# TAMUCrypto/virgo-plus

Measured on AMD Instinct MI355X. Metric: prover sec + field-ops/sec, SHA-256 circuit, 1/2/4/8 MI355X (bit-exact), higher is better.
Workload: dtype u64 (F_p^2, p=2^61-1); 1 GPU; SHA-256 1024-block circuit (SHA256_64.pws x1024, 102347776 gates, 15 layers, 2^23 input wires), GKR sumcheck + Virgo FFT/LDT commit on GPU (BASELINE configs[2]); pass_mode=sync, field_ops_per_proof=8299342697

## Files before the change

### virgo-plus_amd/__init__.py

```python
import ctypes
import os
import shutil
import subprocess

PKG_DIR = os.path.dirname(os.path.abspath(__file__))
ROOT = os.path.dirname(PKG_DIR)
CSRC = os.path.join(PKG_DIR, "csrc")
HOST = os.path.join(PKG_DIR, "host")
LIB_GPU = os.environ.get("VP_LIBGPU") or os.path.join(CSRC, "libvpgpu.so")
LIB_GPU_CHECKED = os.path.join(ROOT, "tools", "_build", "checked", "libvpgpu.so")
LIB_GPU_TESTDRV = os.path.join(ROOT, "tools", "_build", "testdrv", "libvpgpu.so")
LIB_HOST = os.path.join(HOST, "libvphost.so")
CLI = os.path.join(HOST, "virgo_plus_run")

GPU_SRC = [os.path.join(CSRC, f) for f in ("vpgpu.hip", "vpgpu_batched.inc", "vpgpu_pc.inc", "vpgpu_pc_shard.inc", "vpgpu_fftgkr.inc", "vpgpu_upload.inc", "vp_kernels_fftgkr.h", "vp_kernels.h", "vp_kernels_round.h", "vp_kernels_persist.h", "vp_kernels_batch.h",
                                              "vp_kernels_plan.h", "vp_kernels_pc.h", "vp_kernels_ntt8.h", "vp_kernels_ntt_long.h", "vp_keccak_asm.h", "vp_check.h", "vp_field.h", "vp_fri_layout.h", "vp_pc_live.h", "vp_pc_corners.h")] + [
    os.path.join(ROOT, "include", "vpgpu.h")]
HOST_SRC = [os.path.join(HOST, f) for f in ("circuit.cpp", "prover.cpp", "verifier.cpp", "vphost.cpp")]
HOST_HDR = [os.path.join(HOST, f) for f in ("circuit.hpp", "prover.hpp", "verifier.hpp", "vphost.h", "field.hpp",
                                              "polynomial.hpp")]


def _stale(target, sources):
    if not os.path.exists(target):
# ... 547 lines not shown
                                                1 if skip_predicates else 0) == 0

    def verify_full_record(self, record):
        buf = ctypes.create_string_buffer(bytes(record), max(len(record), 1))
        return lib_host().vph_verify_full_record(self.h, ctypes.cast(buf, ctypes.c_void_p), len(record)) == 0

    def verify_fs(self, proof):
        buf = ctypes.create_string_buffer(bytes(proof), len(proof))
        return lib_host().vph_verify_fs(self.h, ctypes.cast(buf, ctypes.c_void_p), len(proof)) == 0

    def close(self):
        if self.h:
            lib_host().vph_circuit_free(self.h)
            self.h = None


_PUBLIC_OPTIONS = ("use_graph", "plan_autotune", "real_values", "real_pairs", "pc_tensor_pub", "persistent_rounds", "persistent_timeout_ms", "poll", "prefetch_round1",
                   "interactive_fast_init", "split_cost_percent", "debug")
_TUNING_ENV = {"gkr_path": "VP_GKR_PATH", "serial": "VP_GKR_SERIAL", "fuse_init": "VP_FUSE_INIT", "fuse_min_log": "VP_FUSE_MIN_LOG", "fuse_dot": "VP_FUSE_DOT",
               "drop_y": "VP_DROP_Y", "drop_y_round1": "VP_DROP_Y1", "seg_tiny": "VP_SEG_TINY", "sf_big_log": "VP_SF_BIG_LOG", "sf3b_grid": "VP_SF3B_GRID",
               "dot_blocks": "VP_DOT_BLOCKS", "plan_align": "VP_PLAN_ALIGN", "round_fused_max": "VP_ROUND_FUSED_MAX",
               "kernel_copies": "VP_KERNEL_COPIES", "fold_branches": "VP_FOLD_BRANCHES", "fuse_combine": "VP_FUSE_COMBINE",
               "graph_explicit": "VP_GRAPH_EXPLICIT", "ntt_r8": "VP_NTT_R8", "fuse_p2": "VP_FUSE_P2", "leaf_asm": "VP_LEAF_ASM",
               "fft_gkr_batched": "VP_FFT_GKR_BATCHED", "split_vu": "VP_SPLIT_VU", "pc_live": "VP_PC_LIVE"}
VP_OPTIONS_ABI = 0x76700005


class Options(ctypes.Structure):
    _fields_ = [("struct_size", ctypes.c_uint32), ("abi", ctypes.c_uint32)] + [(n, ctypes.c_int32) for n in _PUBLIC_OPTIONS] + [("reserved", ctypes.c_int32 * 4)]

    def __init__(self, **kw):
        super().__init__()
        lib_gpu().vp_options_default(ctypes.byref(self))
        self.tuning = {}
        for k, v in kw.items():
            if k in _PUBLIC_OPTIONS:
                setattr(self, k, v)
            elif k in _TUNING_ENV:
                self.tuning[k] = v
            else:
                raise TypeError("unknown option " + k)

    def tuning_env(self):
        env = {}
        for k, v in getattr(self, "tuning", {}).items():
            if k == "gkr_path":
                v = {PATH_PLAN: "plan", PATH_LANES: "lanes", PATH_SIMPLE: "simple"}[v]
# ... 431 lines not shown
```

### virgo-plus_amd/csrc/vp_kernels_ntt8.h

```cpp
#pragma once

namespace vp {

constexpr u64 LZ_P2 = 2 * P61;
constexpr u64 LZ_P4 = 4 * P61;
__device__ __forceinline__ u64 lz_fold(u64 x) { return (x & P61) + (x >> 61); }
__device__ __forceinline__ F lz_fold(const F &x) { return f_make(lz_fold(x.re), lz_fold(x.im)); }
__device__ __forceinline__ F lz_add(const F &a, const F &b) { return f_make(a.re + b.re, a.im + b.im); }
template <u64 K> __device__ __forceinline__ F lz_sub(const F &a, const F &b) { return f_make(a.re + (K - b.re), a.im + (K - b.im)); }
template <bool INV, u64 K> __device__ __forceinline__ F lz_mul_w4(const F &x) { return INV ? f_make(K - x.im, x.re) : f_make(x.im, K - x.re); }
__device__ __forceinline__ u64 lz_rot30(u64 v) { return (v >> 31) + ((v & 0x7fffffffull) << 30); }
template <bool INV> __device__ __forceinline__ F lz_mul_w8(const F &x) {
    const u64 s = x.re + x.im;
    return INV ? f_make(lz_rot30(x.re + (LZ_P2 - x.im)), lz_rot30(s)) : f_make(lz_rot30(s), lz_rot30(x.im + (LZ_P2 - x.re)));
}
__device__ __forceinline__ F lz_canon(const F &x) {
    u64 a = lz_fold(x.re), b = lz_fold(x.im);
    return f_make(a >= P61 ? a - P61 : a, b >= P61 ? b - P61 : b);
}
__device__ __forceinline__ F lz_mul(const F &root, const F &x) { return f_mad31c<true, false>(root, x, f_make(0, 0)); }
__host__ __device__ __forceinline__ F lz_presplit(const F &w) {
    return f_make(((w.re >> 31) << 32) | (w.re & 0x7fffffffull), ((w.im >> 31) << 32) | (w.im & 0x7fffffffull));
}
__device__ __forceinline__ F lz_mul_ps(const F &wp, const F &x) {
// ... 21 lines not shown
    u[2] = lz_fold(lz_add(e2, q2)); u[6] = lz_fold(lz_sub<LZ_P2>(e2, q2));
    u[3] = lz_fold(lz_add(e3, q3)); u[7] = lz_fold(lz_sub<LZ_P2>(e3, q3));
}
template <bool INV> __device__ __forceinline__ void lz_dft4(F (&u)[4]) {
    const F a0 = lz_add(u[0], u[2]), a1 = lz_sub<LZ_P2>(u[0], u[2]), a2 = lz_add(u[1], u[3]), a3 = lz_sub<LZ_P2>(u[1], u[3]);
    const F t3 = lz_mul_w4<INV, LZ_P4>(a3);
    u[0] = lz_fold(lz_add(a0, a2)); u[2] = lz_fold(lz_sub<LZ_P4>(a0, a2)); u[1] = lz_fold(lz_add(a1, t3)); u[3] = lz_fold(lz_sub<LZ_P4>(a1, t3));
}
__device__ __forceinline__ void lz_dft2(F (&u)[2]) {
    const F s = lz_fold(lz_add(u[0], u[1])), d = lz_fold(lz_sub<LZ_P2>(u[0], u[1]));
    u[0] = s; u[1] = d;
}

struct Ntt8Args {
    const F *in; F *out;
    const F *RT; u32 half_m;
    const F *RTn;
    int ln, l1;
    u32 in_stride;
    u32 ncoset;
    int twist;
    int do_scale; F scale;
    const F *in2; u32 pair_rows; const F *e0;
};

constexpr u32 NTT8_TILE = 4096;
constexpr u32 NTT8_THREADS = 512;

template <bool INV>
__global__ void __launch_bounds__(NTT8_THREADS) __attribute__((amdgpu_waves_per_eu(4, 4))) k_ntt8_cols(Ntt8Args a) {
    extern __shared__ __align__(16) unsigned char smem_raw[];
    F *L = reinterpret_cast<F *>(smem_raw);
    const u32 l1 = (u32) a.l1, N1 = 1u << l1, lc = 12 - l1, cols = 1u << lc, N2 = 1u << (a.ln - a.l1), M = 2 * a.half_m;
    const u32 tid = threadIdx.x, row = blockIdx.x, coset = blockIdx.z;
    const u32 c = tid & (cols - 1), j2 = blockIdx.y * cols + c;
    const F *src = a.in + (size_t) row * a.in_stride + j2;
    F *dst = a.out + (((size_t) row * a.ncoset + coset) << a.ln) + j2;
    const u32 wN = M >> a.ln;
    const u32 nr8 = l1 / 3, rem = l1 - 3 * nr8;
    {
        const u32 q = tid >> lc;
        F u[8];
#pragma unroll
        for (u32 m = 0; m < 8; ++m) u[m] = src[(size_t) (q + m * (N1 >> 3)) * N2];
        if (a.in2) {
            const F *src2 = a.in2 + (size_t) row * a.in_stride + j2;
#pragma unroll
            for (u32 m = 0; m < 8; ++m) u[m].im = src2[(size_t) (q + m * (N1 >> 3)) * N2].re;
        }
        if (a.twist && coset) {
            const u32 e0 = q * N2 * coset, step = (N1 >> 3) * N2 * coset;
#pragma unroll
            for (u32 g = 0; g < 8; g += 4) {
                F w[4];
#pragma unroll
                for (u32 m = 0; m < 4; ++m) w[m] = a.RT[(e0 + (g + m) * step) & (M - 1)];
                loads_first();
#pragma unroll
                for (u32 m = 0; m < 4; ++m) u[g + m] = lz_mul(w[m], u[g + m]);
            }
        }
        lz_dft8<INV>(u);
#pragma unroll
        for (u32 m = 0; m < 8; ++m) if (VP_CHK((((q * 8 + m) << lc) + c) < NTT8_TILE, 6, q, m, c)) L[((q * 8 + m) << lc) + c] = u[m];
    }
    __syncthreads();
    u32 s = 8;
    const u32 total_passes = nr8 + (rem ? 1 : 0);
    for (u32 p = 1; p + 1 < total_passes; ++p) {
        const u32 q = tid >> lc, k = q & (s - 1);
        F u[8];
#pragma unroll
        for (u32 m = 0; m < 8; ++m) u[m] = L[((q + m * (N1 >> 3)) << lc) + c];
        {
            const u32 st = N1 / (8 * s);
            F w[8];
#pragma unroll
            for (u32 m = 1; m < 8; ++m) { const u32 e = (k * m * st) & (N1 - 1); w[m] = a.RTn[INV ? ((N1 - e) & (N1 - 1)) : e]; }
#pragma unroll
            for (u32 m = 1; m < 8; ++m) u[m] = lz_mul(w[m], u[m]);
        }
        lz_dft8<INV>(u);
        __syncthreads();
#pragma unroll
        for (u32 m = 0; m < 8; ++m) L[(((q - k) * 8 + k + m * s) << lc) + c] = u[m];
        __syncthreads();
        s *= 8;
    }
    const u32 ec = (a.twist && coset) ? coset : 0u;
    const u32 wNs = INV ? (M - wN) & (M - 1) : wN;
    const u32 ebase = j2 * ec, stepk = j2 * wNs;
    if (rem == 0) {
        const u32 q = tid >> lc, k = q & (s - 1);
        F u[8];
#pragma unroll
        for (u32 m = 0; m < 8; ++m) u[m] = L[((q + m * (N1 >> 3)) << lc) + c];
        {
            const u32 st = N1 / (8 * s);
            F w[8];
#pragma unroll
            for (u32 m = 1; m < 8; ++m) { const u32 e = (k * m * st) & (N1 - 1); w[m] = a.RTn[INV ? ((N1 - e) & (N1 - 1)) : e]; }
#pragma unroll
            for (u32 m = 1; m < 8; ++m) u[m] = lz_mul(w[m], u[m]);
        }
        lz_dft8<INV>(u);
        const u32 k1_0 = (q - k) * 8 + k, eo = ebase + k1_0 * stepk, so = s * stepk;
#pragma unroll
        for (u32 g = 0; g < 8; g += 4) {
            F w[4];
#pragma unroll
            for (u32 m = 0; m < 4; ++m) w[m] = a.RT[(eo + (g + m) * so) & (M - 1)];
            loads_first();
#pragma unroll
            for (u32 m = 0; m < 4; ++m) dst[(size_t) (k1_0 + (g + m) * s) * N2] = lz_mul(w[m], u[g + m]);
        }
    } else if (rem == 2) {
#pragma unroll
        for (u32 h = 0; h < 2; ++h) {
            const u32 t = tid + h * NTT8_THREADS, q = t >> lc, k = q & (s - 1);
            F u[4];
#pragma unroll
            for (u32 m = 0; m < 4; ++m) u[m] = L[((q + m * (N1 >> 2)) << lc) + c];
            const u32 st = N1 / (4 * s);
            F w[4];
#pragma unroll
            for (u32 m = 1; m < 4; ++m) { const u32 e = (k * m * st) & (N1 - 1); w[m] = a.RTn[INV ? ((N1 - e) & (N1 - 1)) : e]; }
#pragma unroll
            for (u32 m = 1; m < 4; ++m) u[m] = lz_mul(w[m], u[m]);
            lz_dft4<INV>(u);
            const u32 k1_0 = (q - k) * 4 + k, eo = ebase + k1_0 * stepk, so = s * stepk;
            F ww[4];
#pragma unroll
            for (u32 m = 0; m < 4; ++m) ww[m] = a.RT[(eo + m * so) & (M - 1)];
            loads_first();
#pragma unroll
            for (u32 m = 0; m < 4; ++m) dst[(size_t) (k1_0 + m * s) * N2] = lz_mul(ww[m], u[m]);
        }
    } else {
#pragma unroll
        for (u32 h = 0; h < 4; ++h) {
            const u32 t = tid + h * NTT8_THREADS, q = t >> lc, k = q & (s - 1);
            F u[2];
            u[0] = L[(q << lc) + c]; u[1] = L[((q + (N1 >> 1)) << lc) + c];
            { const u32 e = k & (N1 - 1); u[1] = lz_mul(a.RTn[INV ? ((N1 - e) & (N1 - 1)) : e], u[1]); }
            lz_dft2(u);
            const u32 k1_0 = (q - k) * 2 + k, eo = ebase + k1_0 * stepk, so = s * stepk;
            F ww[2];
#pragma unroll
            for (u32 m = 0; m < 2; ++m) ww[m] = a.RT[(eo + m * so) & (M - 1)];
            loads_first();
#pragma unroll
            for (u32 m = 0; m < 2; ++m) dst[(size_t) (k1_0 + m * s) * N2] = lz_mul(ww[m], u[m]);
        }
    }
}

struct Ntt8xArgs {
    const F *in; F *out;
    const F *TW;
    const F *T2;
    const F *W1;
    const F *RTn;
    int ln; u32 in_stride, ncoset, cpw;
};
constexpr u32 NTT8X_THREADS = 256, NTT8X_TILE = 2048;
#ifndef VP_NTT8X_WAVES
#define VP_NTT8X_WAVES 2
#endif
#ifndef VP_NTT8X_G
#define VP_NTT8X_G 4
#endif
constexpr u32 NTT8X_G = VP_NTT8X_G;
template <int L1> __device__ __forceinline__ u32 ntt8x_k1(u32 q, u32 o) {
    constexpr u32 Q8 = (1u << L1) >> 3;
    if (L1 == 6) return (q - (q & 7)) * 8 + (q & 7) + o * 8;
// ... 182 lines not shown
```

### virgo-plus_amd/csrc/vpgpu.hip

```cpp
#include <hip/hip_runtime.h>

#include <algorithm>
#include <chrono>
#include <cstdio>
#include <cstring>
#include <deque>
#include <functional>
#include <map>
#include <mutex>
#include <set>
#include <atomic>
#include <string>
#include <thread>
#include <vector>

#include "../../include/vpgpu.h"
#include "vp_kernels.h"
#include "vp_fri_layout.h"
#include "vp_pc_live.h"
#include "vp_pc_corners.h"

using namespace vp;

static_assert(sizeof(vp_F) == sizeof(F), "vp_F layout");
// ... 107 lines not shown
    int32_t drop_y;
    int32_t drop_y_round1;
    int32_t real_values;
    int32_t seg_tiny;
    int32_t sf_big_log;
    int32_t sf3b_grid;
    int32_t dot_blocks;
    int32_t plan_align;
    int32_t round_fused_max;
    int32_t persistent_rounds, poll, debug, prefetch_round1, split_cost_percent;
    int32_t kernel_copies;
    int32_t fold_branches;
    int32_t fuse_combine;
    int32_t plan_autotune, pc_tensor_pub, persistent_timeout_ms;
    int32_t graph_explicit;
    int32_t ntt_r8;
    int32_t interactive_fast_init;
    int32_t fuse_p2;
    int32_t leaf_asm;
    int32_t real_pairs;
    int32_t fft_gkr_batched;
    int32_t split_vu;
    int32_t pc_live;
};

struct vp_ctx {
    int device = 0;
    hipStream_t stream = nullptr;
    std::string err = "";
    int n_layers = 0, max_bl = 0;
    std::vector<LayerDev> L;
    F **d_vals = nullptr;
    unsigned long long **d_valsr = nullptr;
    F *beta_g = nullptr, *beta_u = nullptr, *bf = nullptr, *bs = nullptr, *liu_half = nullptr;
    u32 half_cap = 0;
    F *tab[2][3] = {{nullptr, nullptr, nullptr}, {nullptr, nullptr, nullptr}};
    u32 cap = 0;
    F *partials = nullptr;
    unsigned int *round_arrivals = nullptr;
    F *small = nullptr;
    F *chunk_part = nullptr; u32 chunk_cap = 0;
    F *d_tape = nullptr; u64 n_tape = 0;
    F *d_tr = nullptr; u64 n_tr = 0;
    F *h_pin = nullptr;
    unsigned long long *h_seq = nullptr, seq = 0;
    TailMail *h_req = nullptr; TailReply *h_rep = nullptr; std::atomic<bool> tail_active{false}; unsigned long long tail_seq = 0; int tail_enabled = 1;
// ... 733 lines not shown
    return 0;
#endif
}
const char *vp_version(void) { return "vpgpu 0.1 (gfx950)"; }
const char *vp_last_error(const vp_ctx *ctx) { return ctx ? ctx->err.c_str() : "null context"; }

static void opt_defaults(VpOpt *o) {
    memset(o, 0, sizeof *o);
    o->gkr_path = VP_PATH_PLAN; o->use_graph = 1; o->serial = 0; o->fuse_init = 1; o->fuse_min_log = 0; o->fuse_dot = 0;
    o->drop_y = 1; o->drop_y_round1 = 0; o->real_values = 1; o->seg_tiny = 1; o->sf_big_log = 14;
    o->sf3b_grid = 512; o->dot_blocks = 1024; o->plan_align = 0; o->round_fused_max = 512;
    o->persistent_rounds = 1; o->poll = 1; o->debug = 0; o->prefetch_round1 = 1; o->split_cost_percent = 50; o->kernel_copies = 1; o->fold_branches = 1; o->fuse_combine = 2; o->plan_autotune = 1;
    o->pc_tensor_pub = 1;
    o->persistent_timeout_ms = 10000;
    o->graph_explicit = 0;
    o->ntt_r8 = 1;
    o->interactive_fast_init = 1;
    o->fuse_p2 = 1;
    o->leaf_asm = 1;
    o->real_pairs = 1;
    o->fft_gkr_batched = 1;
    o->split_vu = 1;
    o->pc_live = 1;
}
static void opt_to_public(const VpOpt &o, vp_options *p) {
    memset(p, 0, sizeof *p);
    p->struct_size = (uint32_t) sizeof *p; p->abi = VP_OPTIONS_ABI;
    p->use_graph = o.use_graph; p->plan_autotune = o.plan_autotune; p->real_values = o.real_values; p->real_pairs = o.real_pairs; p->pc_tensor_pub = o.pc_tensor_pub;
    p->persistent_rounds = o.persistent_rounds; p->persistent_timeout_ms = o.persistent_timeout_ms; p->poll = o.poll; p->prefetch_round1 = o.prefetch_round1;
    p->interactive_fast_init = o.interactive_fast_init; p->split_cost_percent = o.split_cost_percent; p->debug = o.debug;
}
void vp_options_default(vp_options *p) {
    if (!p) return;
    VpOpt o; opt_defaults(&o);
    opt_to_public(o, p);
}
int vp_test_drivers(void) {
#ifdef VP_TEST_DRIVERS
    return 1;
#else
    return 0;
#endif
}
struct OptName { const char *name; int32_t VpOpt::*field; };
static const OptName g_opt_names[] = {
    {"gkr_path", &VpOpt::gkr_path}, {"use_graph", &VpOpt::use_graph}, {"serial", &VpOpt::serial}, {"fuse_init", &VpOpt::fuse_init}, {"fuse_min_log", &VpOpt::fuse_min_log},
    {"fuse_dot", &VpOpt::fuse_dot}, {"drop_y", &VpOpt::drop_y}, {"drop_y_round1", &VpOpt::drop_y_round1}, {"real_values", &VpOpt::real_values}, {"seg_tiny", &VpOpt::seg_tiny},
    {"sf_big_log", &VpOpt::sf_big_log}, {"sf3b_grid", &VpOpt::sf3b_grid}, {"dot_blocks", &VpOpt::dot_blocks}, {"plan_align", &VpOpt::plan_align},
    {"round_fused_max", &VpOpt::round_fused_max}, {"persistent_rounds", &VpOpt::persistent_rounds}, {"poll", &VpOpt::poll}, {"debug", &VpOpt::debug},
    {"prefetch_round1", &VpOpt::prefetch_round1}, {"split_cost_percent", &VpOpt::split_cost_percent}, {"kernel_copies", &VpOpt::kernel_copies},
    {"fold_branches", &VpOpt::fold_branches}, {"fuse_combine", &VpOpt::fuse_combine}, {"plan_autotune", &VpOpt::plan_autotune},
    {"pc_tensor_pub", &VpOpt::pc_tensor_pub}, {"persistent_timeout_ms", &VpOpt::persistent_timeout_ms}, {"graph_explicit", &VpOpt::graph_explicit}, {"ntt_r8", &VpOpt::ntt_r8},
    {"interactive_fast_init", &VpOpt::interactive_fast_init}, {"fuse_p2", &VpOpt::fuse_p2}, {"leaf_asm", &VpOpt::leaf_asm},
    {"real_pairs", &VpOpt::real_pairs}, {"fft_gkr_batched", &VpOpt::fft_gkr_batched}, {"split_vu", &VpOpt::split_vu}, {"pc_live", &VpOpt::pc_live}};
int vp_tuning_get(const vp_ctx *ctx, const char *name, int32_t *value) {
    if (!ctx || !name || !value) return VP_EINVAL;
    for (const OptName &n : g_opt_names) if (!strcmp(n.name, name)) { *value = ctx->opt.*(n.field); return VP_OK; }
    return VP_EINVAL;
}
static int resolve_options(VpOpt *o, const vp_options *user, uint32_t *pinned) {
    opt_defaults(o);
    if (user) {
        if (user->struct_size != sizeof(vp_options) || user->abi != VP_OPTIONS_ABI) return VP_EINVAL;
        o->use_graph = user->use_graph; o->plan_autotune = user->plan_autotune; o->real_values = user->real_values; o->real_pairs = user->real_pairs;
        o->pc_tensor_pub = user->pc_tensor_pub; o->persistent_rounds = user->persistent_rounds; o->persistent_timeout_ms = user->persistent_timeout_ms;
        o->poll = user->poll; o->prefetch_round1 = user->prefetch_round1; o->interactive_fast_init = user->interactive_fast_init;
        o->split_cost_percent = user->split_cost_percent; o->debug = user->debug;
    }
    auto flag = [](const char *name, int32_t &v) { const char *e = getenv(name); if (e && (e[0] == '0' || e[0] == '1')) v = e[0] - '0'; };
    auto num = [](const char *name, int32_t &v) { const char *e = getenv(name); if (e && *e) v = atoi(e); };
    if (const char *p = getenv("VP_GKR_PATH"))
        o->gkr_path = !strcmp(p, "lanes") ? VP_PATH_LANES : !strcmp(p, "simple") ? VP_PATH_SIMPLE : VP_PATH_PLAN;
#ifndef VP_TEST_DRIVERS
    if (o->gkr_path != VP_PATH_PLAN) return VP_EINVAL;
#endif
    if (const char *p = getenv("VP_PLAN_ALIGN")) o->plan_align = !strcmp(p, "left") ? 1 : !strcmp(p, "right") ? 2 : 0;
    flag("VP_GKR_GRAPH", o->use_graph); flag("VP_GKR_SERIAL", o->serial); flag("VP_FUSE_INIT", o->fuse_init); flag("VP_FUSE_DOT", o->fuse_dot);
    flag("VP_DROP_Y", o->drop_y); flag("VP_DROP_Y1", o->drop_y_round1); flag("VP_REAL_V", o->real_values);
    flag("VP_SEG_TINY", o->seg_tiny); flag("VP_PERSIST", o->persistent_rounds);
    flag("VP_POLL", o->poll); flag("VP_PREFETCH_R1", o->prefetch_round1);
    num("VP_FUSE_MIN_LOG", o->fuse_min_log); num("VP_SF_BIG_LOG", o->sf_big_log);
    num("VP_SF3B_GRID", o->sf3b_grid); num("VP_DOT_BLOCKS", o->dot_blocks);
    num("VP_ROUND_FUSED_MAX", o->round_fused_max);
    num("VP_SPLIT_COST_PERCENT", o->split_cost_percent);
    flag("VP_KERNEL_COPIES", o->kernel_copies);
    flag("VP_FOLD_BRANCHES", o->fold_branches);
    flag("VP_NTT_R8", o->ntt_r8);
    flag("VP_FAST_INIT", o->interactive_fast_init);
    flag("VP_FUSE_P2", o->fuse_p2);
    flag("VP_LEAF_ASM", o->leaf_asm);
    flag("VP_REAL_PAIRS", o->real_pairs);
    flag("VP_FFT_GKR_BATCHED", o->fft_gkr_batched);
    flag("VP_SPLIT_VU", o->split_vu);
    flag("VP_PC_LIVE", o->pc_live);
    flag("VP_PC_TENSOR", o->pc_tensor_pub);
    num("VP_PERSIST_TIMEOUT_MS", o->persistent_timeout_ms);
    num("VP_GRAPH_EXPLICIT", o->graph_explicit);
    num("VP_FUSE_COMBINE", o->fuse_combine);
    flag("VP_PLAN_AUTOTUNE", o->plan_autotune);
    if (getenv("VP_DEBUG")) o->debug |= 1;
    if (getenv("VP_DEBUG_UPLOAD")) o->debug |= 2;
    o->dot_blocks = std::max(1, o->dot_blocks); o->sf3b_grid = std::max(1, o->sf3b_grid);
    VpOpt d; opt_defaults(&d);
    *pinned = (o->fuse_combine != d.fuse_combine ? 1u : 0u) | (o->fold_branches != d.fold_branches ? 2u : 0u) | (o->plan_align != d.plan_align ? 4u : 0u) |
              (o->fuse_min_log != d.fuse_min_log ? 8u : 0u) | (o->sf3b_grid != d.sf3b_grid ? 16u : 0u) | (o->graph_explicit != d.graph_explicit ? 32u : 0u);
    return VP_OK;
}

int vp_plan_tuning_get(const vp_ctx *ctx, int32_t v[6]) {
    if (!ctx || !v) return VP_EINVAL;
    v[0] = ctx->opt.fuse_combine; v[1] = ctx->opt.fold_branches; v[2] = ctx->opt.plan_align; v[3] = ctx->opt.fuse_min_log; v[4] = ctx->opt.sf3b_grid; v[5] = ctx->opt.graph_explicit;
    return VP_OK;
}
int vp_plan_tuning_set(vp_ctx *ctx, const int32_t v[6]) {
    if (!ctx || !v) return VP_EINVAL;
    if (v[0] < 0 || v[0] > 2 || v[1] < 0 || v[1] > 1 || v[2] < 0 || v[2] > 2 || v[3] < 0 || v[3] > 30 || v[4] < 1 || v[4] > 4096 || v[5] < 0 || v[5] > 3) return VP_EINVAL;
    VP_ENTER(ctx);
// ... 996 lines not shown
```

### virgo-plus_amd/csrc/vpgpu_fftgkr.inc

```
namespace {

struct FgkOffsets {
    int lg; u64 r, x, r0, r1, ru_a, rv_a, ru_m, rv_m, dep0, n;
    explicit FgkOffsets(int lg_) : lg(lg_) {
        r = 0; x = lg; r0 = x + 64; r1 = r0 + lg + 10; ru_a = r1 + lg + 10; rv_a = ru_a + lg + 6; ru_m = rv_a + lg + 6; rv_m = ru_m + lg;
        dep0 = rv_m + lg; n = dep0 + (u64) lg * (2 * lg + 2);
    }
    u64 ru_d(int d) const { return dep0 + (u64) d * (2 * lg + 2); }
    u64 rv_d(int d) const { return ru_d(d) + lg; }
    u64 alpha_d(int d) const { return rv_d(d) + lg; }
    u64 beta_d(int d) const { return alpha_d(d) + 1; }
    static u64 n_msgs(int lg) { return 64 + 3ull * (2ull * lg * lg + 2 * lg + 6) + 2 + 2ull * lg; }
};

}

struct FgkState {
    int lg = 0;
    F *B = nullptr, *S = nullptr, *Pm = nullptr, *winv = nullptr, *sq = nullptr, *xsq = nullptr, *g = nullptr, *eu = nullptr, *hi = nullptr, *part = nullptr, *xt = nullptr;
    F *tape = nullptr, *msgs = nullptr;
    Lane lane;
    std::vector<void *> allocs;
    hipStream_t own_stream = nullptr; hipEvent_t e0 = nullptr, e1 = nullptr, e_dep = nullptr;
    int pending_lg = 0;
// ... 265 lines not shown
    HIPCHK(hipGetLastError());
    memcpy(msgs, s.h_msgs, n_out * sizeof(F));
    float ms = 0;
    hipEventElapsedTime(&ms, s.e0, s.e1);
    ctx->commit_ms = ms;
    if (n_written) *n_written = n_out;
    return VP_OK;
}

int vp_fft_gkr_cancel(vp_ctx *ctx) {
    if (!ctx) return VP_EINVAL;
    VP_ENTER_Q(ctx);
    if (!ctx->fgk || !ctx->fgk->pending_lg) return VP_OK;
    if (ctx->fgk->own_stream) (void) hipStreamSynchronize(ctx->fgk->own_stream);
    ctx->fgk->pending_lg = 0;
    return VP_OK;
}

}

static void warm_kernel_functions() {
    static const void *const fns[] = {
        (const void *) k_ntt8_colsx<6>, (const void *) k_ntt8_colsx<7>, (const void *) k_ntt8_colsx<8>, (const void *) k_ntt8_cols<true>, (const void *) k_ntt8_cols<false>,
        (const void *) k_ntt8_rows<true>, (const void *) k_ntt8_rows<false>, (const void *) k_ntt_lds, (const void *) k_leaf_hash, (const void *) k_leaf_hash_multi,
        (const void *) k_leaf_hash_c, (const void *) k_leaf_hash_multi_c, (const void *) k_leaf_hash_final, (const void *) k_merkle_level, (const void *) k_merkle_top,
        (const void *) k_merkle_level_multi, (const void *) k_merkle_top_multi, (const void *) k_pc_products, (const void *) k_pc_quotient, (const void *) k_pc_rank1_check,
        (const void *) k_pc_dot, (const void *) k_pc_sum_parts, (const void *) k_pc_open, (const void *) k_beta_half, (const void *) k_beta_expand, (const void *) k_zero_f,
        (const void *) k_fri_fold, (const void *) k_fri_fold0_vo, (const void *) k_fri_fold0_vo3<true, VP_VO_GRP>, (const void *) k_fri_fold0_vo3<false, VP_VO_GRP>, (const void *) k_fri_fold0_vo3<true, 1>, (const void *) k_fri_fold0_vo3<false, 1>,
        (const void *) k_fg_pows, (const void *) k_fg_expand, (const void *) k_fg_butterfly, (const void *) k_fg_xsq, (const void *) k_fg_xtab, (const void *) k_fg_polyeval,
        (const void *) k_fg_rowsum, (const void *) k_fg_gtab, (const void *) k_fg_add_init, (const void *) k_fg_mul_init, (const void *) k_fg_gtab_multi, (const void *) k_fg_dot_multi,
        (const void *) k_fg_ifft_multi, (const void *) k_fg_ifft_p1, (const void *) k_fg_ifft_p2, (const void *) k_sumfold3b<true>, (const void *) k_sumfold3b<false>,
        (const void *) k_seg<true>, (const void *) k_seg<false>, (const void *) k_emit,
        (const void *) k_light_multi, (const void *) k_chunks_multi, (const void *) k_combine_multi, (const void *) k_dot_multi, (const void *) k_dotfin_multi,
        (const void *) k_sumfold3b_multi, (const void *) k_sumfold3b_gen_multi, (const void *) k_seg_multi, (const void *) k_emit_multi, (const void *) k_fixup,
        (const void *) k_beta_half_direct, (const void *) k_beta_half_multi, (const void *) k_vres, (const void *) k_vres2, (const void *) k_tape_in, (const void *) k_ship, (const void *) k_ticket,
        (const void *) k_round_main<0>, (const void *) k_round_main<1>, (const void *) k_round_fused, (const void *) k_round_final, (const void *) k_finalize, (const void *) k_phase,
    };
    for (const void *f : fns) { hipFuncAttributes a; (void) hipFuncGetAttributes(&a, f); }
    (void) hipGetLastError();
}
int vp_warm(vp_ctx *ctx, uint32_t what) {
    if (!ctx || !ctx->evaluated) return VP_EINVAL;
    VP_ENTER(ctx);
    if (what) warm_kernel_functions();
    if (what & VP_WARM_COMMITMENT) VPCHK(pc_warm(ctx));
    if (what & VP_WARM_FFT_GKR) {
// ... 26 lines not shown
```

### virgo-plus_amd/csrc/vpgpu_pc.inc

```
namespace {

constexpr int PC_MAX_LN = 13;
#ifndef VP_NTT_SPLIT_LOG
#define VP_NTT_SPLIT_LOG 12
#endif
constexpr int PC_SPLIT_LN = VP_NTT_SPLIT_LOG;

#define PC_PROF(kind, grid, jobs, bytes, work, launch)                                                   \
    do {                                                                                                  \
        const int sl_ = prof_begin(ctx, ctx->stream, (kind), (u32) (grid), (u32) (jobs), (u64) (bytes), (u64) (work)); \
        launch;                                                                                           \
        prof_end(ctx, ctx->stream, sl_);                                                                  \
    } while (0)

F host_pow(F x, unsigned __int128 e) { F r = f_one(); while (e) { if (e & 1) r = f_mul(r, x); x = f_mul(x, x); e >>= 1; } return r; }
F host_root_of_unity(int log_order) {
    F r = f_make(2147483648ull, 1033321771269002680ull);
    for (int i = 0; i < 62 - log_order; ++i) r = f_mul(r, r);
    return r;
}
F host_inv_real(u64 x) { return host_pow(f_make(x, 0), (unsigned __int128) P61 - 2); }

int pc_root_table(vp_ctx *ctx, int lm) {
    if (ctx->pc_lm == lm && ctx->pc_rt) return VP_OK;
// ... 71 lines not shown
    ctx->pc_scr = fresh; ctx->pc_scr_cap = total;
    return VP_OK;
}

#ifndef VP_NTT8X_CHUNK_POW2
#define VP_NTT8X_CHUNK_POW2 1
#endif
#ifndef VP_NTT8X
#define VP_NTT8X 1
#endif
int pc_ntt8x_t2(vp_ctx *ctx, int lm, int ln, int l1, const F **out) {
    const auto key = std::make_pair((const void *) ctx->pc_rt, 1000 + 32 * ln + l1);
    auto it = ctx->pc_rtc.find(key);
    if (it == ctx->pc_rtc.end()) {
        F *t = nullptr;
        const u32 ncoset = 1u << (lm - ln), n2 = 1u << (ln - l1), total = ncoset * n2 * 64;
        VPCHK(dalloc(ctx, &t, (size_t) total));
        hipLaunchKernelGGL(k_ntt8x_t2, dim3(nblk(total)), dim3(VP_BLOCK), 0, ctx->stream, (const F *) ctx->pc_rt, 1u << (lm - 1), (u32) (11 - l1), n2, total, t);
        it = ctx->pc_rtc.emplace(key, t).first;
    }
    *out = it->second;
    return VP_OK;
}
int pc_launch_ntt8(vp_ctx *ctx, const F *in, F *out, int ln, int lm, int inverse, u32 rows, u32 cosets, u32 in_stride, u32 pair_rows = 0) {
    const int l1 = ln - 9;
    const u32 N1 = 1u << l1, nc = inverse ? 1 : cosets;
    const size_t N = (size_t) 1 << ln, total = (size_t) rows * nc * N;
    VPCHK(pc_scratch_reserve(ctx, total));
    const F *rt1 = nullptr, *rt9 = nullptr, *rtm = nullptr;
    VPCHK(pc_circle_roots(ctx, lm, l1, &rt1));
    VPCHK(pc_circle_roots(ctx, lm, 9, &rt9));
    Ntt8Args a{};
    a.in = in; a.out = ctx->pc_scr; a.half_m = 1u << (lm - 1); a.RTn = rt1; a.ln = ln; a.l1 = l1; a.in_stride = in_stride;
    a.ncoset = nc; a.twist = (!inverse && cosets > 1) ? 1 : 0; a.do_scale = 0; a.scale = f_one();
    a.in2 = (pair_rows && inverse) ? in + (size_t) pair_rows * in_stride : nullptr; a.pair_rows = 0; a.e0 = nullptr;
    const u64 tr = (u64) rows * nc;
    const bool colsx = VP_NTT8X && a.twist && l1 >= 6 && l1 <= 8 && cosets == (1u << (lm - ln)) && cosets <= 64;
    Ntt8xArgs x{};
    if (colsx) {
        x.in = in; x.out = ctx->pc_scr; x.RTn = rt1; x.ln = ln; x.in_stride = in_stride; x.ncoset = cosets;
        VPCHK(pc_circle_roots(ctx, lm, l1 + (lm - ln), &x.TW));
        VPCHK(pc_circle_roots(ctx, lm, ln, &x.W1));
        VPCHK(pc_ntt8x_t2(ctx, lm, ln, l1, &x.T2));
        VPCHK(pc_presplit(ctx, x.TW, 1u << (l1 + (lm - ln)), &x.TW));
        VPCHK(pc_presplit(ctx, x.W1, 1u << ln, &x.W1));
        VPCHK(pc_presplit(ctx, x.T2, (1u << (lm - ln)) * (1u << (ln - l1)) * 64u, &x.T2));
        VPCHK(pc_presplit(ctx, x.RTn, 1u << l1, &x.RTn));
    } else {
        VPCHK(pc_circle_roots(ctx, lm, lm, &rtm));
        a.RT = rtm;
    }
    const F *rt9p = nullptr;
    VPCHK(pc_presplit(ctx, rt9, 512u, &rt9p));
    const F *rtz = nullptr;
    const bool pair_fwd = pair_rows && !inverse;
    if (pair_fwd) VPCHK(pc_circle_roots(ctx, lm, lm - ln, &rtz));
    if (ctx->pc_dry) return VP_OK;
    if (colsx) {
        const u32 tiles = (512u << l1) / NTT8X_TILE;
        u32 chunks = 1;
        u32 rows_r = rows;
        if (VP_NTT8X_CHUNK_POW2) { rows_r = 1; while (rows_r < rows) rows_r <<= 1; }
        while (chunks < cosets && (u64) rows_r * tiles * chunks < 8192) chunks <<= 1;
        x.cpw = cosets / chunks;
        const dim3 g(rows, tiles, chunks);
        const int sl_ = prof_begin(ctx, ctx->stream, VP_K_NTT8_COLS, (u32) (g.x * g.y * g.z), (u32) tr, 16ull * N * tr + 16ull * N * rows, tr * (ntt8_cols_mults(ln, 1) + N / 8));
        if (l1 == 6) hipLaunchKernelGGL(k_ntt8_colsx<6>, g, dim3(NTT8X_THREADS), 0, ctx->stream, x);
        else if (l1 == 7) hipLaunchKernelGGL(k_ntt8_colsx<7>, g, dim3(NTT8X_THREADS), 0, ctx->stream, x);
        else hipLaunchKernelGGL(k_ntt8_colsx<8>, g, dim3(NTT8X_THREADS), 0, ctx->stream, x);
        prof_end(ctx, ctx->stream, sl_);
    } else {
        const dim3 g(rows, N1 / 8, nc);
        const int sl_ = prof_begin(ctx, ctx->stream, VP_K_NTT8_COLS, (u32) (g.x * g.y * g.z), (u32) tr, 16ull * N * tr + 16ull * N * rows, tr * ntt8_cols_mults(ln, a.twist));
        if (inverse) hipLaunchKernelGGL(k_ntt8_cols<true>, g, dim3(NTT8_THREADS), NTT8_TILE * sizeof(F), ctx->stream, a);
        else hipLaunchKernelGGL(k_ntt8_cols<false>, g, dim3(NTT8_THREADS), NTT8_TILE * sizeof(F), ctx->stream, a);
        prof_end(ctx, ctx->stream, sl_);
    }
    Ntt8Args b = a;
    b.in = ctx->pc_scr; b.out = out; b.RTn = rt9p; b.do_scale = inverse ? 1 : 0; b.scale = inverse ? host_inv_real(1ull << ln) : f_one();
    b.scale = lz_presplit(b.scale);
    b.in2 = nullptr; b.pair_rows = pair_fwd ? pair_rows : 0; b.e0 = b.pair_rows ? in : nullptr;
    if (b.pair_rows) { b.RT = rtz; b.half_m = nc / 2; }
    {
        const dim3 g(N1 / 8, (u32) tr);
        const int sl_ = prof_begin(ctx, ctx->stream, VP_K_NTT8_ROWS, (u32) (g.x * g.y), (u32) tr, 32ull * N * tr, tr * ntt8_rows_mults(ln, inverse));
        if (inverse) hipLaunchKernelGGL(k_ntt8_rows<true>, g, dim3(NTT8_THREADS), 8 * NTT8_PITCH * sizeof(F), ctx->stream, b);
        else hipLaunchKernelGGL(k_ntt8_rows<false>, g, dim3(NTT8_THREADS), 8 * NTT8_PITCH * sizeof(F), ctx->stream, b);
        prof_end(ctx, ctx->stream, sl_);
    }
    return VP_OK;
}

constexpr int PC_MAX_LN_SPLIT = 17;
constexpr int PC_MAX_LN_LONG = 19;
constexpr int PC_MAX_N = 25;

int pc_launch_ntt_long(vp_ctx *ctx, const F *in, F *out, int ln, int lm, int inverse, u32 rows, u32 cosets, u32 in_stride) {
    const int l0 = ln - PC_MAX_LN_SPLIT, ls = PC_MAX_LN_SPLIT;
    const u32 nc = inverse ? 1 : cosets, N0 = 1u << l0, Ns = 1u << ls;
    const size_t N = (size_t) 1 << ln, total = (size_t) rows * nc * N;
    if ((u64) rows * N0 * nc > 65535) { ctx->err = "transform longer than 2^17 points: more than 65535 sub-transforms in one call"; return VP_ELIMIT; }
    VPCHK(pc_scratch_reserve(ctx, total + (nc > 1 ? total : 0) + (size_t) rows * N));
    F *C = nc > 1 ? ctx->pc_scr + total : out, *D = ctx->pc_scr + total + (nc > 1 ? total : 0);
    const F *rt_sub = nullptr, *W = nullptr;
// ... 422 lines not shown
        else {
            const u32 chk = v.rows_checked();
            HIPCHK(hipMemsetAsync(v.flag, 0, sizeof(int), ctx->stream));
            PC_PROF(VP_K_PC_POINTWISE, nblk((u64) chk * N), 1, 16ull * chk * N, (u64) 2 * chk * N,
                    hipLaunchKernelGGL(k_pc_rank1_check, dim3(nblk((u64) chk * N)), dim3(VP_BLOCK), 0, ctx->stream, (const F *) v.slice0, N, chk, v.flag));
            int bad = 1;
            HIPCHK(hipMemcpyAsync(&bad, v.flag, sizeof(int), hipMemcpyDeviceToHost, ctx->stream));
            HIPCHK(hipStreamSynchronize(ctx->stream));
            v.tensor = bad == 0;
        }
    }
    if (v.tensor) {
        F *sc = nullptr;
        VPCHK(ring_alloc(ctx, 64 * sizeof(F), (void **) &sc));
        const F inv0 = host_pow(corner[0], (unsigned __int128) P61 * P61 - 2);
        for (int i = 0; i < 64; ++i) sc[i] = f_mul(corner[i], inv0);
        HIPCHK(hipMemcpyAsync(v.qscal(), sc, 64 * sizeof(F), hipMemcpyHostToDevice, ctx->stream));
        VPCHK(pc_launch_ntt(ctx, v.slice0, v.coef, ln, lm, 1, 1, 1, N));
        VPCHK(pc_launch_ntt(ctx, v.coef, v.q0, ln, lm, 0, 1, 32, N));
    } else {
        VPCHK(pc_launch_ntt(ctx, v.pub, v.coef, ln, lm, 1, rows, 1, N));
        VPCHK(pc_launch_ntt(ctx, v.coef, v.qcw, ln, lm, 0, rows, 32, N));
    }
    PC_PROF(VP_K_PC_POINTWISE, nblk((u64) 2 * rows * N), 1, 48ull * 2 * rows * N, (u64) 2 * rows * N,
            hipLaunchKernelGGL(k_pc_products, dim3(nblk((u64) 2 * rows * N)), dim3(VP_BLOCK), 0, ctx->stream, v.lcw, v.qcw, N, v.P(), rows, v.q0_arg(), v.qs_arg()));
    VPCHK(pc_launch_ntt(ctx, v.P(), v.ST(), ln, lm, 1, 2 * rows, 1, N));
    hipLaunchKernelGGL(k_zero_f, dim3(1), dim3(256), 0, ctx->stream, v.d_all(), 144u);
    PC_PROF(VP_K_PC_POINTWISE, nblk((u64) rows * N), 1, 48ull * rows * N, (u64) 2 * rows * N,
            hipLaunchKernelGGL(k_pc_quotient, dim3(nblk((u64) rows * N)), dim3(VP_BLOCK), 0, ctx->stream, v.ST(), N, ctx->pc_rt, M >> 1,
                               host_inv_real(2), f_make(N, 0), v.H(), v.d_all(), rows));
    return pc_launch_ntt(ctx, v.H(), v.hcw, ln, lm, 0, rows, 32, N);
}

int pc_commit_public_body(vp_ctx *ctx, hipEvent_t &ev_a, const F corner[64], int tensor_state, vp_F *inner, vp_F all_sum[65], uint8_t root_h[32],
                          const vp_F *pub_mask = nullptr, uint64_t n_pub_mask = 0) {
    const int n = ctx->L[0].bl, lm = n - 1;
    const u32 N = 1u << (n - 6), M = 1u << lm;
    VPCHK(pc_hash_outstanding(ctx, 2u));
    if (!pub_mask) VPCHK(pc_live_zero_hcw(ctx));
    const bool late = ctx->hash_late && !pub_mask;
    PcSlices v = pc_slices(ctx, pub_mask ? 64u : ctx->pc_lv.live);
    F *d_inner = v.d_inner(), *d_all = v.d_all();
    const u32 used = (u32) ctx->L[0].size, g = std::min<u32>(1024, nblk(used));
    PC_PROF(VP_K_PC_POINTWISE, g, 1, 32ull * used, used, hipLaunchKernelGGL(k_pc_dot, dim3(g), dim3(VP_BLOCK), 0, ctx->stream, ctx->L[0].val, ctx->pc_pub, used, v.small));
    hipLaunchKernelGGL(k_pc_sum_parts, dim3(1), dim3(VP_BLOCK), 0, ctx->stream, v.small, g, d_inner);
    VPCHK(pc_quotient_slices(ctx, v, corner, tensor_state));
    ctx->pc_q_tensor = v.tensor;
    const u32 n_leaves = M >> 1;
    if (pub_mask) {
// ... 630 lines not shown
```

Baseline: 167.8 billion field-ops/s.

## Fuse PC pointwise products into compact inverse NTT column pass

Adds compact modes to the inverse radix-8 column NTT kernel. Mode 1 computes output twiddles from a presplit length-N root table instead of the full length-M table. Modes 2 and 3 form the lcw*qcw (or scaled q0) products while loading, so the separate k_pc_products kernel and its intermediate buffer round trip are no longer needed. The fused mode runs only for ln in [13,17] with r8 enabled. It risks correctness if the compact twiddle indexing does not match the original and adds more kernel variants to maintain.

Result: no change. 168.1 billion field-ops/s (median of 3 runs) (+0.1%).

```diff
diff --git a/virgo-plus_amd/__init__.py b/virgo-plus_amd/__init__.py
--- a/virgo-plus_amd/__init__.py
+++ b/virgo-plus_amd/__init__.py
@@ -593,7 +593,7 @@
                "dot_blocks": "VP_DOT_BLOCKS", "plan_align": "VP_PLAN_ALIGN", "round_fused_max": "VP_ROUND_FUSED_MAX",
                "kernel_copies": "VP_KERNEL_COPIES", "fold_branches": "VP_FOLD_BRANCHES", "fuse_combine": "VP_FUSE_COMBINE",
                "graph_explicit": "VP_GRAPH_EXPLICIT", "ntt_r8": "VP_NTT_R8", "fuse_p2": "VP_FUSE_P2", "leaf_asm": "VP_LEAF_ASM",
-               "fft_gkr_batched": "VP_FFT_GKR_BATCHED", "split_vu": "VP_SPLIT_VU", "pc_live": "VP_PC_LIVE"}
+               "fft_gkr_batched": "VP_FFT_GKR_BATCHED", "split_vu": "VP_SPLIT_VU", "pc_live": "VP_PC_LIVE", "inv_chain": "VP_INV_CHAIN"}
 VP_OPTIONS_ABI = 0x76700005
 
 
diff --git a/virgo-plus_amd/csrc/vp_kernels_ntt8.h b/virgo-plus_amd/csrc/vp_kernels_ntt8.h
--- a/virgo-plus_amd/csrc/vp_kernels_ntt8.h
+++ b/virgo-plus_amd/csrc/vp_kernels_ntt8.h
@@ -67,33 +67,53 @@
     int twist;
     int do_scale; F scale;
     const F *in2; u32 pair_rows; const F *e0;
+    const F *W1;
+    const F *lcw, *qcw, *q0, *qscal;
 };
 
 constexpr u32 NTT8_TILE = 4096;
 constexpr u32 NTT8_THREADS = 512;
 
-template <bool INV>
+template <bool INV, int MODE = 0>
 __global__ void __launch_bounds__(NTT8_THREADS) __attribute__((amdgpu_waves_per_eu(4, 4))) k_ntt8_cols(Ntt8Args a) {
+    static_assert(MODE == 0 || INV, "the compact forms are the inverse's");
     extern __shared__ __align__(16) unsigned char smem_raw[];
     F *L = reinterpret_cast<F *>(smem_raw);
     const u32 l1 = (u32) a.l1, N1 = 1u << l1, lc = 12 - l1, cols = 1u << lc, N2 = 1u << (a.ln - a.l1), M = 2 * a.half_m;
     const u32 tid = threadIdx.x, row = blockIdx.x, coset = blockIdx.z;
     const u32 c = tid & (cols - 1), j2 = blockIdx.y * cols + c;
     const F *src = a.in + (size_t) row * a.in_stride + j2;
-    F *dst = a.out + (((size_t) row * a.ncoset + coset) << a.ln) + j2;
+    F *dst = MODE ? nullptr : a.out + (((size_t) row * a.ncoset + coset) << a.ln) + j2;
     const u32 wN = M >> a.ln;
     const u32 nr8 = l1 / 3, rem = l1 - 3 * nr8;
     {
         const u32 q = tid >> lc;
         F u[8];
-#pragma unroll
-        for (u32 m = 0; m < 8; ++m) u[m] = src[(size_t) (q + m * (N1 >> 3)) * N2];
-        if (a.in2) {
+        if constexpr (MODE >= 2) {
+            const u32 i = row >> 1, b = (row & 1) ? 16u : 0u;
+            const size_t cs = ((size_t) i * 32 + b) << a.ln;
+            const F *lb = a.lcw + cs;
+            const F *qb = MODE == 3 ? a.q0 + ((size_t) b << a.ln) : a.qcw + cs;
+            const F sc = MODE == 3 ? a.qscal[i] : f_one();
+#pragma unroll
+            for (u32 g = 0; g < 8; g += 4) {
+                F l[4], qq[4];
+#pragma unroll
+                for (u32 m = 0; m < 4; ++m) { const u32 o = (q + (g + m) * (N1 >> 3)) * N2 + j2; l[m] = lb[o]; qq[m] = qb[o]; }
+                loads_first();
+#pragma unroll
+                for (u32 m = 0; m < 4; ++m) u[g + m] = f_mul(l[m], MODE == 3 ? f_mul(sc, qq[m]) : qq[m]);
+            }
+        } else {
+#pragma unroll
+            for (u32 m = 0; m < 8; ++m) u[m] = src[(size_t) (q + m * (N1 >> 3)) * N2];
+        }
+        if (MODE < 2 && a.in2) {
             const F *src2 = a.in2 + (size_t) row * a.in_stride + j2;
 #pragma unroll
             for (u32 m = 0; m < 8; ++m) u[m].im = src2[(size_t) (q + m * (N1 >> 3)) * N2].re;
         }
-        if (a.twist && coset) {
+        if (MODE == 0 && a.twist && coset) {
             const u32 e0 = q * N2 * coset, step = (N1 >> 3) * N2 * coset;
 #pragma unroll
             for (u32 g = 0; g < 8; g += 4) {
@@ -132,9 +152,11 @@
         __syncthreads();
         s *= 8;
     }
+    if constexpr (MODE != 0) dst = a.out + ((size_t) row << a.ln) + j2;
     const u32 ec = (a.twist && coset) ? coset : 0u;
     const u32 wNs = INV ? (M - wN) & (M - 1) : wN;
     const u32 ebase = j2 * ec, stepk = j2 * wNs;
+    const u32 NM = (1u << a.ln) - 1;
     if (rem == 0) {
         const u32 q = tid >> lc, k = q & (s - 1);
         F u[8];
@@ -154,10 +176,10 @@
         for (u32 g = 0; g < 8; g += 4) {
             F w[4];
 #pragma unroll
-            for (u32 m = 0; m < 4; ++m) w[m] = a.RT[(eo + (g + m) * so) & (M - 1)];
+            for (u32 m = 0; m < 4; ++m) w[m] = MODE ? a.W1[(0u - j2 * (k1_0 + (g + m) * s)) & NM] : a.RT[(eo + (g + m) * so) & (M - 1)];
             loads_first();
 #pragma unroll
-            for (u32 m = 0; m < 4; ++m) dst[(size_t) (k1_0 + (g + m) * s) * N2] = lz_mul(w[m], u[g + m]);
+            for (u32 m = 0; m < 4; ++m) dst[(size_t) (k1_0 + (g + m) * s) * N2] = MODE ? lz_mul_ps(w[m], u[g + m]) : lz_mul(w[m], u[g + m]);
         }
     } else if (rem == 2) {
 #pragma unroll
@@ -176,10 +198,10 @@
             const u32 k1_0 = (q - k) * 4 + k, eo = ebase + k1_0 * stepk, so = s * stepk;
             F ww[4];
 #pragma unroll
-            for (u32 m = 0; m < 4; ++m) ww[m] = a.RT[(eo + m * so) & (M - 1)];
+            for (u32 m = 0; m < 4; ++m) ww[m] = MODE ? a.W1[(0u - j2 * (k1_0 + m * s)) & NM] : a.RT[(eo + m * so) & (M - 1)];
             loads_first();
 #pragma unroll
-            for (u32 m = 0; m < 4; ++m) dst[(size_t) (k1_0 + m * s) * N2] = lz_mul(ww[m], u[m]);
+            for (u32 m = 0; m < 4; ++m) dst[(size_t) (k1_0 + m * s) * N2] = MODE ? lz_mul_ps(ww[m], u[m]) : lz_mul(ww[m], u[m]);
         }
     } else {
 #pragma unroll
@@ -192,10 +214,10 @@
             const u32 k1_0 = (q - k) * 2 + k, eo = ebase + k1_0 * stepk, so = s * stepk;
             F ww[2];
 #pragma unroll
-            for (u32 m = 0; m < 2; ++m) ww[m] = a.RT[(eo + m * so) & (M - 1)];
+            for (u32 m = 0; m < 2; ++m) ww[m] = MODE ? a.W1[(0u - j2 * (k1_0 + m * s)) & NM] : a.RT[(eo + m * so) & (M - 1)];
             loads_first();
 #pragma unroll
-            for (u32 m = 0; m < 2; ++m) dst[(size_t) (k1_0 + m * s) * N2] = lz_mul(ww[m], u[m]);
+            for (u32 m = 0; m < 2; ++m) dst[(size_t) (k1_0 + m * s) * N2] = MODE ? lz_mul_ps(ww[m], u[m]) : lz_mul(ww[m], u[m]);
         }
     }
 }
diff --git a/virgo-plus_amd/csrc/vpgpu.hip b/virgo-plus_amd/csrc/vpgpu.hip
--- a/virgo-plus_amd/csrc/vpgpu.hip
+++ b/virgo-plus_amd/csrc/vpgpu.hip
@@ -153,6 +153,7 @@
     int32_t fft_gkr_batched;
     int32_t split_vu;
     int32_t pc_live;
+    int32_t inv_chain;
 };
 
 struct vp_ctx {
@@ -932,6 +933,7 @@
     o->fft_gkr_batched = 1;
     o->split_vu = 1;
     o->pc_live = 1;
+    o->inv_chain = 1;
 }
 static void opt_to_public(const VpOpt &o, vp_options *p) {
     memset(p, 0, sizeof *p);
@@ -962,7 +964,7 @@
     {"fold_branches", &VpOpt::fold_branches}, {"fuse_combine", &VpOpt::fuse_combine}, {"plan_autotune", &VpOpt::plan_autotune},
     {"pc_tensor_pub", &VpOpt::pc_tensor_pub}, {"persistent_timeout_ms", &VpOpt::persistent_timeout_ms}, {"graph_explicit", &VpOpt::graph_explicit}, {"ntt_r8", &VpOpt::ntt_r8},
     {"interactive_fast_init", &VpOpt::interactive_fast_init}, {"fuse_p2", &VpOpt::fuse_p2}, {"leaf_asm", &VpOpt::leaf_asm},
-    {"real_pairs", &VpOpt::real_pairs}, {"fft_gkr_batched", &VpOpt::fft_gkr_batched}, {"split_vu", &VpOpt::split_vu}, {"pc_live", &VpOpt::pc_live}};
+    {"real_pairs", &VpOpt::real_pairs}, {"fft_gkr_batched", &VpOpt::fft_gkr_batched}, {"split_vu", &VpOpt::split_vu}, {"pc_live", &VpOpt::pc_live}, {"inv_chain", &VpOpt::inv_chain}};
 int vp_tuning_get(const vp_ctx *ctx, const char *name, int32_t *value) {
     if (!ctx || !name || !value) return VP_EINVAL;
     for (const OptName &n : g_opt_names) if (!strcmp(n.name, name)) { *value = ctx->opt.*(n.field); return VP_OK; }
@@ -1003,6 +1005,7 @@
     flag("VP_FFT_GKR_BATCHED", o->fft_gkr_batched);
     flag("VP_SPLIT_VU", o->split_vu);
     flag("VP_PC_LIVE", o->pc_live);
+    flag("VP_INV_CHAIN", o->inv_chain);
     flag("VP_PC_TENSOR", o->pc_tensor_pub);
     num("VP_PERSIST_TIMEOUT_MS", o->persistent_timeout_ms);
     num("VP_GRAPH_EXPLICIT", o->graph_explicit);
diff --git a/virgo-plus_amd/csrc/vpgpu_fftgkr.inc b/virgo-plus_amd/csrc/vpgpu_fftgkr.inc
--- a/virgo-plus_amd/csrc/vpgpu_fftgkr.inc
+++ b/virgo-plus_amd/csrc/vpgpu_fftgkr.inc
@@ -311,6 +311,7 @@
 static void warm_kernel_functions() {
     static const void *const fns[] = {
         (const void *) k_ntt8_colsx<6>, (const void *) k_ntt8_colsx<7>, (const void *) k_ntt8_colsx<8>, (const void *) k_ntt8_cols<true>, (const void *) k_ntt8_cols<false>,
+        (const void *) k_ntt8_cols<true, 1>, (const void *) k_ntt8_cols<true, 2>, (const void *) k_ntt8_cols<true, 3>,
         (const void *) k_ntt8_rows<true>, (const void *) k_ntt8_rows<false>, (const void *) k_ntt_lds, (const void *) k_leaf_hash, (const void *) k_leaf_hash_multi,
         (const void *) k_leaf_hash_c, (const void *) k_leaf_hash_multi_c, (const void *) k_leaf_hash_final, (const void *) k_merkle_level, (const void *) k_merkle_top,
         (const void *) k_merkle_level_multi, (const void *) k_merkle_top_multi, (const void *) k_pc_products, (const void *) k_pc_quotient, (const void *) k_pc_rank1_check,
diff --git a/virgo-plus_amd/csrc/vpgpu_pc.inc b/virgo-plus_amd/csrc/vpgpu_pc.inc
--- a/virgo-plus_amd/csrc/vpgpu_pc.inc
+++ b/virgo-plus_amd/csrc/vpgpu_pc.inc
@@ -117,7 +117,8 @@
     *out = it->second;
     return VP_OK;
 }
-int pc_launch_ntt8(vp_ctx *ctx, const F *in, F *out, int ln, int lm, int inverse, u32 rows, u32 cosets, u32 in_stride, u32 pair_rows = 0) {
+struct PcProd { const F *lcw, *qcw, *q0, *qscal; };
+int pc_launch_ntt8(vp_ctx *ctx, const F *in, F *out, int ln, int lm, int inverse, u32 rows, u32 cosets, u32 in_stride, u32 pair_rows = 0, const PcProd *prod = nullptr) {
     const int l1 = ln - 9;
     const u32 N1 = 1u << l1, nc = inverse ? 1 : cosets;
     const size_t N = (size_t) 1 << ln, total = (size_t) rows * nc * N;
@@ -131,6 +132,8 @@
     a.in2 = (pair_rows && inverse) ? in + (size_t) pair_rows * in_stride : nullptr; a.pair_rows = 0; a.e0 = nullptr;
     const u64 tr = (u64) rows * nc;
     const bool colsx = VP_NTT8X && a.twist && l1 >= 6 && l1 <= 8 && cosets == (1u << (lm - ln)) && cosets <= 64;
+    const bool compact = inverse && ctx->opt.inv_chain;
+    if (prod && !compact) { ctx->err = "pc_launch_ntt8: products on the load need the compact inverse"; return VP_EINVAL; }
     Ntt8xArgs x{};
     if (colsx) {
         x.in = in; x.out = ctx->pc_scr; x.RTn = rt1; x.ln = ln; x.in_stride = in_stride; x.ncoset = cosets;
@@ -141,6 +144,10 @@
         VPCHK(pc_presplit(ctx, x.W1, 1u << ln, &x.W1));
         VPCHK(pc_presplit(ctx, x.T2, (1u << (lm - ln)) * (1u << (ln - l1)) * 64u, &x.T2));
         VPCHK(pc_presplit(ctx, x.RTn, 1u << l1, &x.RTn));
+    } else if (compact) {
+        VPCHK(pc_circle_roots(ctx, lm, ln, &a.W1));
+        VPCHK(pc_presplit(ctx, a.W1, 1u << ln, &a.W1));
+        if (prod) { a.in = prod->lcw; a.lcw = prod->lcw; a.qcw = prod->qcw; a.q0 = prod->q0; a.qscal = prod->qscal; }
     } else {
         VPCHK(pc_circle_roots(ctx, lm, lm, &rtm));
         a.RT = rtm;
@@ -167,7 +174,10 @@
     } else {
         const dim3 g(rows, N1 / 8, nc);
         const int sl_ = prof_begin(ctx, ctx->stream, VP_K_NTT8_COLS, (u32) (g.x * g.y * g.z), (u32) tr, 16ull * N * tr + 16ull * N * rows, tr * ntt8_cols_mults(ln, a.twist));
-        if (inverse) hipLaunchKernelGGL(k_ntt8_cols<true>, g, dim3(NTT8_THREADS), NTT8_TILE * sizeof(F), ctx->stream, a);
+        if (prod && prod->q0) hipLaunchKernelGGL((k_ntt8_cols<true, 3>), g, dim3(NTT8_THREADS), NTT8_TILE * sizeof(F), ctx->stream, a);
+        else if (prod) hipLaunchKernelGGL((k_ntt8_cols<true, 2>), g, dim3(NTT8_THREADS), NTT8_TILE * sizeof(F), ctx->stream, a);
+        else if (compact) hipLaunchKernelGGL((k_ntt8_cols<true, 1>), g, dim3(NTT8_THREADS), NTT8_TILE * sizeof(F), ctx->stream, a);
+        else if (inverse) hipLaunchKernelGGL(k_ntt8_cols<true>, g, dim3(NTT8_THREADS), NTT8_TILE * sizeof(F), ctx->stream, a);
         else hipLaunchKernelGGL(k_ntt8_cols<false>, g, dim3(NTT8_THREADS), NTT8_TILE * sizeof(F), ctx->stream, a);
         prof_end(ctx, ctx->stream, sl_);
     }
@@ -175,6 +185,7 @@
     b.in = ctx->pc_scr; b.out = out; b.RTn = rt9p; b.do_scale = inverse ? 1 : 0; b.scale = inverse ? host_inv_real(1ull << ln) : f_one();
     b.scale = lz_presplit(b.scale);
     b.in2 = nullptr; b.pair_rows = pair_fwd ? pair_rows : 0; b.e0 = b.pair_rows ? in : nullptr;
+    b.W1 = nullptr; b.lcw = b.qcw = b.q0 = b.qscal = nullptr;
     if (b.pair_rows) { b.RT = rtz; b.half_m = nc / 2; }
     {
         const dim3 g(N1 / 8, (u32) tr);
@@ -643,9 +654,14 @@
         VPCHK(pc_launch_ntt(ctx, v.pub, v.coef, ln, lm, 1, rows, 1, N));
         VPCHK(pc_launch_ntt(ctx, v.coef, v.qcw, ln, lm, 0, rows, 32, N));
     }
-    PC_PROF(VP_K_PC_POINTWISE, nblk((u64) 2 * rows * N), 1, 48ull * 2 * rows * N, (u64) 2 * rows * N,
-            hipLaunchKernelGGL(k_pc_products, dim3(nblk((u64) 2 * rows * N)), dim3(VP_BLOCK), 0, ctx->stream, v.lcw, v.qcw, N, v.P(), rows, v.q0_arg(), v.qs_arg()));
-    VPCHK(pc_launch_ntt(ctx, v.P(), v.ST(), ln, lm, 1, 2 * rows, 1, N));
+    if (ctx->opt.inv_chain && ctx->opt.ntt_r8 && ln >= 13 && ln <= PC_MAX_LN_SPLIT && (u64) 2 * rows <= 65535) {
+        const PcProd pr{v.lcw, v.qcw, v.q0_arg(), v.qs_arg()};
+        VPCHK(pc_launch_ntt8(ctx, nullptr, v.ST(), ln, lm, 1, 2 * rows, 1, N, 0, &pr));
+    } else {
+        PC_PROF(VP_K_PC_POINTWISE, nblk((u64) 2 * rows * N), 1, 48ull * 2 * rows * N, (u64) 2 * rows * N,
+                hipLaunchKernelGGL(k_pc_products, dim3(nblk((u64) 2 * rows * N)), dim3(VP_BLOCK), 0, ctx->stream, v.lcw, v.qcw, N, v.P(), rows, v.q0_arg(), v.qs_arg()));
+        VPCHK(pc_launch_ntt(ctx, v.P(), v.ST(), ln, lm, 1, 2 * rows, 1, N));
+    }
     hipLaunchKernelGGL(k_zero_f, dim3(1), dim3(256), 0, ctx->stream, v.d_all(), 144u);
     PC_PROF(VP_K_PC_POINTWISE, nblk((u64) rows * N), 1, 48ull * rows * N, (u64) 2 * rows * N,
             hipLaunchKernelGGL(k_pc_quotient, dim3(nblk((u64) rows * N)), dim3(VP_BLOCK), 0, ctx->stream, v.ST(), N, ctx->pc_rt, M >> 1,
```
